# BetterBelle/eco-dqn

Measured on NVIDIA B200. Metric: env-steps/sec incl. MPNN Q-eval, higher is better.
Workload: dtype bf16x2-split/f32

## Files before the change

### eco-dqn_b200/csrc/env_step_device.cuh

```cuda
#pragma once
#include <limits.h>

#include "eco_common.cuh"

namespace eco {

union V8s { uint2 v; int8_t b[8]; };
union V8h { uint4 v; int16_t h[8]; };
union V8u { uint4 v; uint16_t h[8]; };
union V4s { uint32_t v; int8_t b[4]; };
union V4h { uint2 v; int16_t h[4]; };
union V4u { uint2 v; uint16_t h[4]; };

__device__ __forceinline__ float feat_gain(int gain, double mlr) {
    return (float)__ddiv_rn((double)gain, mlr);
}

struct SmallDiv {
    float m, y;
    bool ok;
};
__device__ __forceinline__ SmallDiv small_div_setup(double mlr, bool integer_couplings) {
    SmallDiv d;
    d.m = (float)mlr;
    d.ok = integer_couplings && mlr != 0.0 && fabs(mlr) <= 2048.0;
    d.y = __frcp_rn(d.ok ? d.m : 1.f);
    return d;
}
__device__ __forceinline__ float small_div(float a, const SmallDiv& d) {
    const float q0 = __fmul_rn(a, d.y);
    const float r = __fmaf_rn(-q0, d.m, a);
    return __fmaf_rn(r, d.y, q0);
}
__device__ __forceinline__ uint32_t prmt(uint32_t a, uint32_t b, uint32_t sel) {
    uint32_t r;
    asm("prmt.b32 %0, %1, %2, %3;" : "=r"(r) : "r"(a), "r"(b), "r"(sel));
    return r;
}
__device__ __forceinline__ int sx8(uint32_t w, int k) { return (int)prmt(w, 0, k | ((8 | k) << 4) | ((8 | k) << 8) | ((8 | k) << 12)); }
__device__ __forceinline__ int sx16(uint32_t w, int hh) {
    return (int)prmt(w, 0, (2 * hh) | ((2 * hh + 1) << 4) | ((8 | (2 * hh + 1)) << 8) | ((8 | (2 * hh + 1)) << 12));
}
__device__ __forceinline__ int zx16(uint32_t w, int hh) { return (int)prmt(w, 0, (2 * hh) | ((2 * hh + 1) << 4) | 0x4400); }

struct StepScalars {
    double score, nscore, best_score, best_nscore, rew;
    int n_visited;
    bool new_best;
};
__device__ __forceinline__ StepScalars bls_step_scalars(const eco_env_t& env, const double (&sc)[4], double delta,
                                                        double delta_n, int nimp, int n_visited, uint64_t* tab, uint32_t slot,
                                                        ulonglong2 tv, uint64_t k0, uint64_t k1) {
    StepScalars r;
    r.score = __dadd_rn(sc[0], delta);
    r.nscore = __dadd_rn(sc[1], delta_n);
    r.rew = 0.0;
    if (r.score > sc[2]) r.rew = __dsub_rn(r.nscore, sc[3]);
    if (env.use_basin) {
        const uint64_t w0 = k0 ^ VISITED_SALT0, w1 = k1 ^ VISITED_SALT1;
        bool is_new = false;
        for (int probe = 0; probe < env.HCAP; ++probe) {
            if (tv.x == 0 && tv.y == 0) {
                *reinterpret_cast<ulonglong2*>(tab + 2 * slot) = make_ulonglong2(w0, w1);
                is_new = true; ++n_visited;
                break;
            }
            if (tv.x == w0 && tv.y == w1) break;
            slot = (slot + 1) & (env.HCAP - 1);
            tv = *reinterpret_cast<const ulonglong2*>(tab + 2 * slot);
        }
        if (nimp == 0 && is_new) r.rew = __dadd_rn(r.rew, env.basin_reward);
    }
    r.n_visited = n_visited;
    r.new_best = r.score > sc[2];
    r.best_score = r.new_best ? r.score : sc[2];
    r.best_nscore = r.new_best ? r.nscore : sc[3];
    return r;
}

template <int TPE, bool WIDE = true>
__device__ __forceinline__ void env_step_group(const eco_graphs_t& g, const eco_env_t& env, long long b, const int lane,
                                               const bool in_range, const int policy, const int action,
                                               double* __restrict__ reward_out, uint8_t* __restrict__ done_out,
                                               int32_t* __restrict__ hist_a, double* __restrict__ hist_r,
                                               double* __restrict__ hist_s) {
    const int N = env.N, NP = env.NP, NCH = NP >> 3;
    const bool has = lane < NCH;

    eco_episode_t* ep = env.ep + b;
    const int4 e0 = *reinterpret_cast<const int4*>(ep);
    const int4 e1 = *(reinterpret_cast<const int4*>(ep) + 1);
    const int gi = env.graph_idx[b];
    int a = policy == ECO_POLICY_GREEDY ? 0 : action;
    int8_t* spins = env.spins + (size_t)b * NP;
    int16_t* hf = env.hfield + (size_t)b * NP;
    uint16_t* lf = env.last_flip + (size_t)b * NP;
    V8s s; V8h h; V8u l;
    s.v = make_uint2(0, 0); h.v = make_uint4(0, 0, 0, 0); l.v = make_uint4(0, 0, 0, 0);
    if (has) {
        s.v = *reinterpret_cast<const uint2*>(spins + lane * 8);
        h.v = *reinterpret_cast<const uint4*>(hf + lane * 8);
        l.v = *reinterpret_cast<const uint4*>(lf + lane * 8);
    }
    double sc[4] = {0, 0, 0, 0};
    ulonglong2 key = make_ulonglong2(0, 0);
    double total_reward = 0.0;
    if (lane == 0) {
        const double2 d0 = *reinterpret_cast<const double2*>(&ep->score);
        const double2 d1 = *reinterpret_cast<const double2*>(&ep->best_score);
        sc[0] = d0.x; sc[1] = d0.y; sc[2] = d1.x; sc[3] = d1.y;
        key = *reinterpret_cast<const ulonglong2*>(&ep->key[0]);
        total_reward = ep->total_reward;
    }
    const int flags = e1.y;
    const int step_new = e0.x + 1;
    bool active = in_range && !(flags & (FLAG_DONE | FLAG_STOPPED)) && step_new <= env.T;

    if (policy == ECO_POLICY_GREEDY) {
        int best = INT_MIN;
#pragma unroll
        for (int k = 0; k < 8; ++k) {
            const int i = lane * 8 + k;
            if (has && i < N)
                best = max(best, (int)((((uint32_t)(s.b[k] * h.h[k] + 32768) << 16) | (uint32_t)(0xFFFF - i)) ^ 0x80000000u));
        }
        best = group_max<TPE>(best);
        const uint32_t ukey = (uint32_t)best ^ 0x80000000u;
        a = 0xFFFF - (int)(ukey & 0xFFFFu);
        if (active && ((int)(ukey >> 16) - 32768) < 0) {
            active = false;
            if (lane == 0) ep->flags = flags | FLAG_STOPPED;
        }
    }
    if (a < 0 || a >= N) { a = 0; active = false; }

    V8s j;
    j.v = make_uint2(0, 0);
    if (has && active) j.v = *reinterpret_cast<const uint2*>(g.J + ((size_t)gi * NP + a) * NP + lane * 8);
    const double mlr = g.gscal[(size_t)gi * 4 + 0];
    const bool use_tab = (g.reserved & ECO_GRAPHS_PM1) != 0;
    const float* gtab = g.gain_tab + (size_t)gi * tab_stride(NP) + NP;
    double qn = 1.0;
    ulonglong2 zob = make_ulonglong2(0, 0);
    uint32_t old_word = 0;
    if (lane == 0) {
        if (!use_tab) qn = g.gscal[(size_t)gi * 4 + 1];
        zob = *reinterpret_cast<const ulonglong2*>(env.zobrist + 2 * a);
        old_word = env.diff_bits[(size_t)b * env.NW + (a >> 5)];
    }
    const int ka = a & 7;
    const uint32_t sw = ka < 4 ? s.v.x : s.v.y;
    const int my_s = (int)(int8_t)(sw >> (8 * (ka & 3)));
    const uint32_t hw = ka < 2 ? h.v.x : (ka < 4 ? h.v.y : (ka < 6 ? h.v.z : h.v.w));
    const int my_h = (int)(int16_t)(hw >> (16 * (ka & 1)));
    const int s_a_old = __shfl_sync(0xffffffffu, my_s, a >> 3, TPE);
    const int h_a_old = __shfl_sync(0xffffffffu, my_h, a >> 3, TPE);
    const int s_a_new = -s_a_old;

    const uint64_t k0 = key.x ^ zob.x, k1 = key.y ^ zob.y;
    uint64_t* tab = env.visited + (size_t)b * env.HCAP * 2;
    uint32_t slot = (uint32_t)(k0 ^ (k0 >> 29)) & (env.HCAP - 1);
    ulonglong2 tv = make_ulonglong2(0, 0);
    const int delta = s_a_old * h_a_old;
    double delta_n = 0.0;
    if (lane == 0 && active) {
        if (env.use_basin) tv = *reinterpret_cast<const ulonglong2*>(tab + 2 * slot);
        if (use_tab) delta_n = __ldg(g.dn_tab + (size_t)gi * tab_stride(NP) + NP + delta);
    }

    int nimp = 0;
    if (has && active) {
        float* x0 = env.xn + (size_t)b * 3 * NP + lane * 8;
        auto vertex = [&](int k, float& o0, float& o1, float& o2) {
            const int i = lane * 8 + k;
            int si = s.b[k];
            if (i == a) { si = s_a_new; s.b[k] = (int8_t)si; l.h[k] = (uint16_t)step_new; }
            const int hi = h.h[k] + 2 * j.b[k] * s_a_new;
            h.h[k] = (int16_t)hi;
            const int gain = si * hi;
            nimp += gain > 0;
            o0 = (float)si;
            o1 = use_tab ? __ldg(gtab + gain) : feat_gain(gain, mlr);
            o2 = __ldg(env.tsf_tab + (step_new - l.h[k]));
        };
        if (WIDE) {
            float f0[8], f1[8], f2[8];
#pragma unroll
            for (int k = 0; k < 8; ++k) vertex(k, f0[k], f1[k], f2[k]);
            st_f32x8(x0, f0);
            st_f32x8(x0 + NP, f1);
            st_f32x8(x0 + 2 * NP, f2);
        } else {
#pragma unroll
            for (int half = 0; half < 2; ++half) {
                float f0[4], f1[4], f2[4];
#pragma unroll
                for (int kk = 0; kk < 4; ++kk) vertex(half * 4 + kk, f0[kk], f1[kk], f2[kk]);
                *reinterpret_cast<float4*>(x0 + 4 * half) = make_float4(f0[0], f0[1], f0[2], f0[3]);
                *reinterpret_cast<float4*>(x0 + NP + 4 * half) = make_float4(f1[0], f1[1], f1[2], f1[3]);
// ... 53 lines not shown
```

### eco-dqn_b200/csrc/mpnn_tc.cu

```cuda
#include <cuda_bf16.h>
#include <stdlib.h>

#include "eco_common.cuh"
#include "tc_prims.cuh"
#include "mpnn_pack.cuh"
#include "env_step_device.cuh"

namespace eco {
namespace {

using namespace tc;

constexpr int NPMAX = 208;
constexpr int PACK_NPMAX = 192;
constexpr int CHUNK = 64;
constexpr int SUBS = 2;
constexpr int THREADS = 256 * SUBS;
constexpr int GROUP_THREADS = 128 * SUBS;
constexpr int NWARPS = THREADS / 32;
constexpr int ISSUERS = 4;
constexpr int LAUNCH_THREADS = THREADS + 32 * ISSUERS;

constexpr uint32_t T_ACC0 = 0;
constexpr uint32_t T_ACC1 = 208;
// ... 116 lines not shown
}

__device__ __forceinline__ void store_block(const Ctx& c, unsigned char* buf, int node0, const float (&v)[8]) {
    const int rowoff = 16 * (c.lane >> 2) + 4 * (c.lane & 3);
#pragma unroll
    for (int half = 0; half < 2; ++half) {
        const int cb = (node0 >> 3) + half;
#pragma unroll
        for (int fr = 0; fr < 2; ++fr) {
            uint32_t hi, lo;
            split2(v[4 * half + 2 * fr], v[4 * half + 2 * fr + 1], hi, lo);
            unsigned char* p = buf + ((cb * 16 + 4 * c.q + fr) * 128) + rowoff;
            *reinterpret_cast<uint32_t*>(p) = hi;
            *reinterpret_cast<uint32_t*>(p + 2 * 128) = lo;
        }
    }
}

__device__ __forceinline__ void issue_part(const Ctx& c, uint32_t acc_col, uint32_t tw, const unsigned char* x, int cb0,
                                           int width , bool accumulate) {
    const uint32_t idesc = instr_desc_bf16(128, width, false, true);
    const uint32_t idesc_lo = instr_desc_bf16(64, width, false, true);
    const uint64_t d = smem_desc(smem_u32(x) + cb0 * 2048,  128,  2048);
#pragma unroll
    for (int i = 0; i < 8; ++i)
        mma_ts(c.tmem + acc_col, c.tmem + tw + 8 * (i >> 1), d + (uint64_t)(16 * i), (i & 1) ? idesc_lo : idesc, accumulate || i > 0);
}

struct FusedEnv {
    eco_env_t env;
    int32_t* hist_a;
    double* hist_r;
    double* hist_s;
    int n_steps;
};

template <bool PACKED, bool TLINE, bool FUSED = false>
__global__ void __launch_bounds__(LAUNCH_THREADS, 1)
mpnn_tc_kernel(const eco_graphs_t g, const eco_mpnn_t w, const int B, const int32_t* __restrict__ graph_idx,
               const float* __restrict__ xn, const float* __restrict__ xg, const float norm_max,
               float* __restrict__ q_out, int32_t* __restrict__ act_out, unsigned long long* __restrict__ dbg,
               const int packK, const FusedEnv fe) {
    extern __shared__ __align__(128) unsigned char smem[];
    int dbg_n = 0;
#define TL(id)                                                                                           \
    do {                                                                                                 \
        if (TLINE && dbg != nullptr && blockIdx.x == 0 && (threadIdx.x & 31) == 0 && dbg_n < 1024)       \
            dbg[(threadIdx.x >> 5) * 1024 + dbg_n++] = ((unsigned long long)(id) << 48) | (clock64() & 0xFFFFFFFFFFFFull); \
    } while (0)
    __shared__ uint64_t bars[9];
    __shared__ uint64_t sig[2];
    __shared__ uint64_t sdbar[4];
    __shared__ uint64_t tail_sig, tail_done;
    __shared__ uint64_t gsig[2][2];
    __shared__ uint64_t bar_ops[2];
    __shared__ uint32_t tmem_base_s;
    Ctx c;
    c.smem = smem; c.phase_all = 0; c.phase_grp = 0; c.phase_g2 = 0; c.phase_g3 = 0;
    c.tid = threadIdx.x; c.lane = c.tid & 31;
    c.warp = __shfl_sync(0xffffffffu, c.tid >> 5, 0);
    c.q = c.warp & 3; c.sub = (c.warp >> 2) % SUBS;
    c.grp = c.warp < NWARPS ? c.warp / (4 * SUBS) : (c.warp == NWARPS + 2 ? 1 : 0);
    const bool linear_issuer = c.warp == NWARPS + 1 || c.warp == NWARPS + 2;
    c.bar_all = &bars[0]; c.bar_grp = &bars[1 + c.grp]; c.bar_g2 = &bars[5 + c.grp]; c.bar_g3 = &bars[7 + c.grp];
    const int K = PACKED ? packK : 1;
    const int NPs = g.NP, Ns = g.N;
    c.NP = K * NPs; c.NB = c.NP >> 3; c.N = PACKED ? c.NP : g.N;
    const int N = c.N, NP = c.NP, NB = c.NB;
    const int N8 = PACKED ? NP : ((N + 7) & ~7);
    const int npacks = (B + K - 1) / K;
    const int n_e = (int)blockIdx.x < npacks ? (npacks - (int)blockIdx.x + (int)gridDim.x - 1) / (int)gridDim.x : 0;
    const int n_items = n_e * (FUSED ? fe.n_steps : 1);
    auto item_ep = [&](int it) { return (int)blockIdx.x + (FUSED ? it % n_e : it) * (int)gridDim.x; };
    auto vertex_ok = [&](int n) { return PACKED ? (n % NPs) < Ns : n < N; };
    float* rdmaxv = reinterpret_cast<float*>(smem + SM_A + PACK_NPMAX * PACK_NPMAX * 2);
    float* pp_blk = rdmaxv + PACK_NPMAX;
    float* pooled_e = pp_blk + (PACK_NPMAX / 16) * 64;
    float* tef = pooled_e + (PACK_NPMAX / 16) * 64;

    float* xf = reinterpret_cast<float*>(smem + SM_XF);
    float* rdeg = reinterpret_cast<float*>(smem + SM_DEG);
    float* qpart = reinterpret_cast<float*>(smem + SM_QP);
    float* ppart = reinterpret_cast<float*>(smem + SM_PP);
    float* pooled = ppart;
    float* s_c0 = reinterpret_cast<float*>(smem + SM_MISC);
    float* red_val = s_c0 + 16;
    int* red_idx = reinterpret_cast<int*>(s_c0 + 32);
    unsigned char* sA = smem + SM_A;
    unsigned char* sAbs = smem + SM_ABS;
    unsigned char* sH = smem + SM_H;
    unsigned char* sE = smem + SM_E;
    unsigned char* sT = smem + SM_T + c.grp * (128 * CHUNK * 2);
    const uint32_t acc1 = T_ACC1 + 64 * c.grp;
    const uint32_t* pk = reinterpret_cast<const uint32_t*>(w.packed);

    if (c.warp == 0) tmem_alloc(&tmem_base_s, 512);
    if (c.tid == 0) {
        for (int i = 0; i < 9; ++i) mbar_init(&bars[i], 1);
        mbar_init(&bar_ops[0], 1); mbar_init(&bar_ops[1], 1);
        mbar_init(&sig[0], 1); mbar_init(&sig[1], 1);
        for (int i = 0; i < 4; ++i) mbar_init(&gsig[i >> 1][i & 1], 4 * SUBS);
        for (int i = 0; i < 4; ++i) mbar_init(&sdbar[i], NWARPS);
        mbar_init(&tail_sig, 1); mbar_init(&tail_done, 1);
        fence_mbar_init();
    }
    tc_fence_before();
    __syncthreads();
    tc_fence_after();
    c.tmem = tmem_base_s;
    if (c.warp < 4 && N8 < NP) {
        const uint32_t z[8] = {0, 0, 0, 0, 0, 0, 0, 0};
        tmem_st_32x32b_x8(tmem_addr(c.tmem, 32 * c.q, T_ACC0 + N8), z);
        tmem_st_wait();
        tc_fence_before();
    }
    const float dmax_set = norm_max > 0.f ? norm_max : *g.dmax;
    const int nsteps_A = NP >> 4;
    const int nblocks = NP >> 4;
    const int nb0 = group0_blocks(nblocks), nb1 = nblocks - nb0;
    const int nch0 = nb0 >= 2 ? 2 : nb0, nch1 = nb1 >= 2 ? 2 : nb1;
    const int nchunks = nch0 + nch1;
    const int chunk_split = nch0;
    const int cs = c.grp == 0 ? 0 : nch0;
    const int ncols0 = 16 * nb0;
    uint32_t phase_half = 0, phase_other = 0, phase_tail = 0;
    const int nmine = (c.warp < NWARPS || linear_issuer) ? (c.grp == 0 ? nch0 : nch1) : 0;
    const int nbm = c.grp == 0 ? nb0 : nb1;
    const int cA0 = c.grp == 0 ? 0 : ncols0, cAw = nmine > 1 ? 16 * ((nbm + 1) / 2) : 16 * nbm;
    const int cB0 = cA0 + cAw, cBw = 16 * nbm - cAw;
    const int cAm = min(cAw, N8 - cA0), cBm = min(cBw, N8 - cB0);
    auto signal_issuer = [&](int k) {
        fence_proxy_async();
        tc_fence_before();
        __syncwarp();
        if (c.lane == 0) mbar_arrive(&gsig[c.grp][k & 1]);
    };

// ... 88 lines not shown
            for (int j = 0; j < 16; ++j) {
                const float pv = pooled[k0 + 2 * j + kpar];
                acc.x = fmaf(a[j].x, pv, acc.x); acc.y = fmaf(a[j].y, pv, acc.y);
                acc.z = fmaf(a[j].z, pv, acc.z); acc.w = fmaf(a[j].w, pv, acc.w);
            }
        }
        acc.x += __shfl_xor_sync(0xffffffffu, acc.x, 16); acc.y += __shfl_xor_sync(0xffffffffu, acc.y, 16);
        acc.z += __shfl_xor_sync(0xffffffffu, acc.z, 16); acc.w += __shfl_xor_sync(0xffffffffu, acc.w, 16);
        const float4 wr = __ldg(reinterpret_cast<const float4*>(w.w_read + f4));
        float t = kpar == 0 ? fmaf(wr.x, fmaxf(acc.x, 0.f), fmaf(wr.y, fmaxf(acc.y, 0.f),
                              fmaf(wr.z, fmaxf(acc.z, 0.f), wr.w * fmaxf(acc.w, 0.f)))) : 0.f;
#pragma unroll
        for (int o = 16; o > 0; o >>= 1) t += __shfl_xor_sync(0xffffffffu, t, o);
        TL(62);
        return bread + t;
    };
    auto readout_warp_b = [&](const int be, const float c0v) {
        TL(63);
        float bv = -INFINITY;
        int bi = 0x7fffffff;
        for (int i = c.lane; i < N; i += 32) {
            const float qv = c0v + ((qpart[i] + qpart[NPMAX + i]) + (qpart[2 * NPMAX + i] + qpart[3 * NPMAX + i]));
            if (q_out) q_out[(size_t)be * NP + i] = qv;
            if (qv > bv) { bv = qv; bi = i; }
        }
#pragma unroll
        for (int o = 16; o > 0; o >>= 1) {
            const float ov = __shfl_xor_sync(0xffffffffu, bv, o);
            const int oi = __shfl_xor_sync(0xffffffffu, bi, o);
            if (ov > bv || (ov == bv && oi < bi)) { bv = ov; bi = oi; }
        }
        if (c.lane == 0 && act_out) act_out[be] = bi;
        if (FUSED)
            env_step_group<32, false>(g, fe.env, be, c.lane, true, ECO_POLICY_ACTIONS, bi, nullptr, nullptr, fe.hist_a, fe.hist_r, fe.hist_s);
        TL(64);
    };
    constexpr int XF_DEG = 4, XF_GL = 5, XF_GMAX = 6;
    float* wsm_e = xf + 7 * NPMAX;
    float* wsm_i = wsm_e + 63 * 8;
    auto stage_inputs = [&](int e) {
        const int i = c.tid - GROUP_THREADS, per_row = NP >> 2;
        const int ge = graph_idx[e];
        if (i < 4 * per_row) {
            const int row = i / per_row, col = 4 * (i % per_row);
            const float* src = row < 3 ? xn + ((size_t)e * 3 + row) * NP + col : g.deg + (size_t)ge * NP + col;
            float* dst = xf + (row < 3 ? row : XF_DEG) * NPMAX + col;
            asm volatile("cp.async.cg.shared.global [%0], [%1], 16;" ::"r"(smem_u32(dst)), "l"(src) : "memory");
        } else if (i == 4 * per_row) {
            asm volatile("cp.async.cg.shared.global [%0], [%1], 16;" ::"r"(smem_u32(xf + XF_GL * NPMAX)), "l"(xg + (size_t)e * 4) : "memory");
        } else if (i == 4 * per_row + 1) {
            asm volatile("cp.async.ca.shared.global [%0], [%1], 4;" ::"r"(smem_u32(xf + XF_GMAX * NPMAX)), "l"(g.gstat + (size_t)ge * 4) : "memory");
        }
        if (i < (63 * 8) / 4)
            asm volatile("cp.async.ca.shared.global [%0], [%1], 16;" ::"r"(smem_u32(wsm_e + 4 * i)), "l"(w.w_edge + 4 * i) : "memory");
        if (i < (64 * 7) / 4)
            asm volatile("cp.async.ca.shared.global [%0], [%1], 16;" ::"r"(smem_u32(wsm_i + 4 * i)), "l"(w.w_init + 4 * i) : "memory");
        asm volatile("cp.async.commit_group;" ::: "memory");
    };
    auto readout_packed_warp = [&](const int be) {
        TL(60);
        const int bpe = NPs >> 4;
        for (int idx = c.lane; idx < K * 64; idx += 32) {
            const int e = idx >> 6, f = idx & 63;
            float t = 0.f;
            for (int j = 0; j < bpe; ++j) t += pp_blk[(e * bpe + j) * 64 + f];
            pooled_e[idx] = t / (float)Ns;
        }
        __syncwarp();
        TL(61);
        constexpr int KMAX = PACK_NPMAX / 16;
        float p0[KMAX], p1[KMAX];
#pragma unroll
        for (int e = 0; e < KMAX; ++e) { p0[e] = 0.f; p1[e] = 0.f; }
        const float* wt = reinterpret_cast<const float*>(pk + PK_WPT) + c.lane;
#pragma unroll 1
        for (int k0 = 0; k0 < 64; k0 += 16) {
            float wa[16], wb[16];
#pragma unroll
            for (int j = 0; j < 16; ++j) { wa[j] = __ldg(wt + (k0 + j) * 64); wb[j] = __ldg(wt + (k0 + j) * 64 + 32); }
#pragma unroll
            for (int j = 0; j < 16; ++j) {
#pragma unroll
                for (int e = 0; e < KMAX; ++e) {
                    if (e < K) {
                        const float pv = pooled_e[e * 64 + k0 + j];
                        p0[e] = fmaf(wa[j], pv, p0[e]);
                        p1[e] = fmaf(wb[j], pv, p1[e]);
                    }
                }
            }
        }
// ... 19 lines not shown
            const int ep = be * K + e;
            const float c0v = pooled_e[e];
            for (int v = c.lane; v < NPs; v += 32) {
                const int i = i0 + v;
                const float qv = c0v + ((qpart[i] + qpart[NPMAX + i]) + (qpart[2 * NPMAX + i] + qpart[3 * NPMAX + i]));
                const bool ok = v < Ns && ep < B;
                if (ok && q_out) q_out[(size_t)ep * NPs + v] = qv;
                qpart[i] = ok ? qv : -INFINITY;
            }
        }
        __syncwarp();
        TL(65);
        for (int e = 0; e < K; ++e) {
            const int ep = be * K + e;
            float bv = -INFINITY;
            int bi = 0x7fffffff;
            for (int v = c.lane; v < Ns; v += 32) {
                const float qv = qpart[e * NPs + v];
                if (qv > bv) { bv = qv; bi = v; }
            }
#pragma unroll
            for (int o = 16; o > 0; o >>= 1) {
                const float ov = __shfl_xor_sync(0xffffffffu, bv, o);
                const int oi = __shfl_xor_sync(0xffffffffu, bi, o);
                if (ov > bv || (ov == bv && oi < bi)) { bv = ov; bi = oi; }
            }
            if (c.lane == 0 && ep < B && act_out) act_out[ep] = bi;
        }
        TL(64);
    };
    if (c.warp == NWARPS) {

        uint32_t sp0 = 0, sp1 = 0, sp2 = 0, op = 0;
        for (int it = 0; it < n_items; ++it) {
            mbar_wait(&bar_ops[0], op);
            mbar_wait(&bar_ops[1], op); op ^= 1u;
            TL(51);
            for (int r = 0; 4 * r < nsteps_A; ++r) {
                mbar_wait(&sdbar[r], sp0);
                tc_fence_after();
                if (r == 0) TL(50);
                if (elect_one()) {
                    const uint32_t idesc = instr_desc_bf16(128, N8, false, false);
                    const uint64_t bd_abs = smem_desc(smem_u32(sAbs), NB * 128, 128);
                    const uint64_t bd_a = smem_desc(smem_u32(sA), NB * 128, 128);
                    const uint64_t kstep = (uint64_t)((2 * NB * 128) >> 4);
                    for (int ks = 4 * r; ks < min(4 * r + 4, nsteps_A); ++ks) {
                        mma_ts(c.tmem + T_ACC0, c.tmem + T_S + 8 * ks, bd_abs + ks * kstep, idesc, ks > 0);
                        mma_ts(c.tmem + T_ACC0, c.tmem + T_D + 8 * ks, bd_a + ks * kstep, idesc, true);
                    }
                    if (4 * r + 4 >= nsteps_A) mma_commit(c.bar_all);
                }
                __syncwarp();
            }
            sp0 ^= 1u;
            TL(52);
            for (int l = 0; l < 3; ++l) {
                mbar_wait(&sig[1], sp1); sp1 ^= 1u;
                tc_fence_after();
                TL(53);
                if (elect_one()) {
                    const uint64_t ad = smem_desc(smem_u32(sH), 2048, 128);
                    const uint64_t bstep = (uint64_t)((2 * NB * 128) >> 4);
                    for (int half = 0; half < 2; ++half) {
                        const int n0 = half ? ncols0 : 0, ncols = half ? N8 - ncols0 : min(ncols0, N8);
                        if (ncols == 0) break;
                        const uint32_t idesc = instr_desc_bf16(128, ncols, false, false);
                        const uint64_t bd = smem_desc(smem_u32(sA) + (n0 >> 3) * 128, NB * 128, 128);
                        for (int ks = 0; ks < nsteps_A; ++ks)
                            mma_ss(c.tmem + T_ACC0 + n0, ad + (uint64_t)ks * (4096 >> 4), bd + ks * bstep, idesc, ks > 0);
                        mma_commit(&bars[3 + half]);
                    }
                }
                __syncwarp();
                TL(54);
            }
            if (PACKED && it + 1 < n_items) {
                mbar_wait(&bars[N8 > ncols0 ? 4 : 3], (uint32_t)((3 * it + 2) & 1));
                fetch_ops_warp(0, item_ep(it + 1));
                mbar_wait(&sig[0], sp2); sp2 ^= 1u;
                fetch_ops_warp(1, item_ep(it + 1));
            }
        }
    }
    if (c.warp == NWARPS + 3) {
        uint32_t ph = 0;
        for (int it = 0; it < n_items - (PACKED ? 1 : 0); ++it) {
            mbar_wait(&tail_sig, ph);
            ph ^= 1u;
            if (PACKED) readout_packed_warp(item_ep(it));
            else readout_warp_b(item_ep(it), readout_warp_a());
            if (FUSED) __threadfence();
            __syncwarp();
            if (c.lane == 0) mbar_arrive(&tail_done);
        }
    }
    if (linear_issuer && nmine > 0) {
        uint32_t ph[2] = {0, 0};
        auto wait_sig = [&](int k) {
            mbar_wait(&gsig[c.grp][k & 1], ph[k & 1]);
            ph[k & 1] ^= 1u;
            tc_fence_after();
        };
        for (int it = 0; it < n_items; ++it) {
            wait_sig(0);
            if (elect_one()) { issue_part(c, T_ACC0 + cA0, T_WEF, sE, cA0 >> 3, cAm, false); mma_commit(c.bar_grp); }
            __syncwarp();
            if (nmine > 1) {
                wait_sig(1);
                if (elect_one()) { issue_part(c, acc1, T_WEF, sE, cB0 >> 3, cBm, false); mma_commit(c.bar_g2); }
                __syncwarp();
            }
            for (int l = 0; l < 3; ++l) {
                wait_sig(0);
                if (elect_one()) issue_part(c, acc1, T_WM + 32, sE, cA0 >> 3, cAm, false);
                __syncwarp();
                wait_sig(1);
                if (elect_one()) {
                    issue_part(c, acc1, T_WM, sT, 0, cAm, true);
                    mma_commit(c.bar_grp);
                    issue_part(c, T_ACC0 + cA0, T_WU, sH, cA0 >> 3, cAm, false);
                    mma_commit(c.bar_g2);
                }
                __syncwarp();
                if (nmine > 1) {
                    wait_sig(0);
                    if (elect_one()) {
                        issue_part(c, T_ACC0 + cB0, T_WU, sH, cB0 >> 3, cBm, false);
                        mma_commit(c.bar_g3);
                    }
                    __syncwarp();
                }
                wait_sig(1);
                if (elect_one()) {
                    issue_part(c, T_ACC0 + cA0, T_WU + 32, sH, cA0 >> 3, cAm, true);
                    mma_commit(c.bar_grp);
                    if (nmine > 1) {
// ... 45 lines not shown
            workers_sync();
            if (c.tid < NP) {
                const int i = c.tid, e = i / NPs, v = i % NPs, ep = be * K + e;
                float c0v = bread;
                for (int f = 0; f < 64; ++f) c0v += tef[e * 64 + f];
                const float qv = c0v + ((qpart[i] + qpart[NPMAX + i]) + (qpart[2 * NPMAX + i] + qpart[3 * NPMAX + i]));
                const bool ok = v < Ns && ep < B;
                if (ok && q_out) q_out[(size_t)ep * NPs + v] = qv;
                qpart[i] = ok ? qv : -INFINITY;
            }
            workers_sync();
            for (int e = c.warp; e < K; e += NWARPS) {
                const int ep = be * K + e;
                float bv = -INFINITY;
                int bi = 0x7fffffff;
                for (int v = c.lane; v < Ns; v += 32) {
                    const float qv = qpart[e * NPs + v];
                    if (qv > bv) { bv = qv; bi = v; }
                }
#pragma unroll
                for (int o = 16; o > 0; o >>= 1) {
                    const float ov = __shfl_xor_sync(0xffffffffu, bv, o);
                    const int oi = __shfl_xor_sync(0xffffffffu, bi, o);
                    if (ov > bv || (ov == bv && oi < bi)) { bv = ov; bi = oi; }
                }
                if (c.lane == 0 && ep < B && act_out) act_out[ep] = bi;
            }
            workers_sync();
            return;
        }
    };
    int last_b = -1;

    for (int it = 0; it < n_items && c.warp < NWARPS; ++it) {
        const int b = item_ep(it);
        const bool has_next = it + 1 < n_items;
        const int b_next = has_next ? item_ep(it + 1) : 0;
        TL(1);
        if (!PACKED) {
            asm volatile("cp.async.wait_group 0;" ::: "memory");
            TL(70);
            workers_sync();
            TL(71);
            gl = *reinterpret_cast<const float4*>(xf + XF_GL * NPMAX);
            gmaxdeg = *reinterpret_cast<const int*>(xf + XF_GMAX * NPMAX);
            if (has_v) rdeg[c.tid] = __fdividef(1.f, xf[XF_DEG * NPMAX + c.tid]);
        }
        const float rdmax = __fdividef(1.f, norm_max < 0.f ? (float)max(gmaxdeg, 1) : dmax_set);

        const int fa = 16 * c.q + (c.lane >> 2), fb = fa + 8;
        float wxa[8], wxb[8], wia[7], wib[7];
        {
            const float* we = PACKED ? w.w_edge : wsm_e;
            const float* wi = PACKED ? w.w_init : wsm_i;
#pragma unroll
            for (int k = 0; k < 8; ++k) {
                wxa[k] = we[fa * 8 + k];
                wxb[k] = fb < 63 ? we[fb * 8 + k] : 0.f;
            }
#pragma unroll
            for (int k = 0; k < 7; ++k) { wia[k] = wi[fa * 7 + k]; wib[k] = wi[fb * 7 + k]; }
        }
        if (PACKED && has_v) {
            const int i = c.tid;
            const bool ok = vertex_ok(i);
            xf[0 * NPMAX + i] = ok ? xin0 : 0.f;
            xf[1 * NPMAX + i] = ok ? xin1 : 0.f;
            xf[2 * NPMAX + i] = ok ? xin2 : 0.f;
            rdeg[i] = __fdividef(1.f, degv);
            {
                xf[3 * NPMAX + i] = ok ? gl.x : 0.f;
                xf[4 * NPMAX + i] = ok ? gl.y : 0.f;
                xf[5 * NPMAX + i] = ok ? gl.z : 0.f;
                xf[6 * NPMAX + i] = ok ? gl.w : 0.f;
                rdmaxv[i] = 1.f / (norm_max < 0.f ? (float)max(gmaxdeg, 1) : dmax_set);
            }
// ... 116 lines not shown
                store_block(c, sE, c0 + bc, v);
            });
        };
        if (nmine > 0) {
            TL(15);
            wait_grp(c);
            TL(12);
            epi_e(T_ACC0, cA0, cA0, cAw);
            TL(13);
        }

        auto epi_agg = [&](int c0, int width, bool wait_b1) {
            bool waited = !wait_b1;
            epilogue(c, T_ACC0, c0, width, [&](int bc, float (&v)[8]) {
                const int n0 = c0 + bc + 2 * (c.lane & 3);
                const float2 r0 = *reinterpret_cast<const float2*>(rdeg + n0), r1 = *reinterpret_cast<const float2*>(rdeg + n0 + 8);
                const float rd[4] = {r0.x, r0.y, r1.x, r1.y};
#pragma unroll
                for (int i = 0; i < 8; i += 2) mul2(v[i], v[i + 1], v[i], v[i + 1], rd[2 * (i >> 2)], rd[2 * (i >> 2) + 1]);
                if (!waited) { wait_grp(c); waited = true; }
                store_block(c, sT, bc, v);
            });
            if (!waited) wait_grp(c);
        };
        auto epi_m = [&](int c0, int width) {
            epilogue(c, acc1, 0, width, [&](int bc, float (&v)[8]) {
#pragma unroll
                for (int i = 0; i < 8; ++i) v[i] = fmaxf(v[i], 0.f);
                store_block(c, sH, c0 + bc, v);
            });
        };
        for (int l = 0; l < 3; ++l) {
            TL(20);
            cta_stage_sync();
            TL(21);
            if (c.tid == 0) mbar_arrive(&sig[1]);
            if (l > 0) {
                uint4 wm[64 / (8 * SUBS)], wu[64 / (8 * SUBS)];
                ldg_weights<64>(c, pk + PK_WM + l * 128 * 64, wm);
                ldg_weights<64>(c, pk + PK_WU + l * 128 * 64, wu);
                sttm_weights<64>(c, wm, T_WM);
                sttm_weights<64>(c, wu, T_WU);
                tmem_st_wait();
                tc_fence_before();
                workers_sync();
            }
            if (l == 0 && nmine > 1) {
                wait_g2(c);
                epi_e(acc1, 0, cB0, cBw);
                TL(13);
            }
            if (nmine > 0) signal_issuer(0);
            TL(22);
            float wa = 0.f, wb = 0.f;
            if (l == 2) { wa = __ldg(w.w_read + 64 + fa); wb = __ldg(w.w_read + 64 + fa + 8); }
            if (l == 2 && last_b >= 0) {
                mbar_wait(&tail_done, phase_tail);
                phase_tail ^= 1u;
            }
            if (nmine > 0) {
                mbar_wait(&bars[3 + c.grp], phase_half);
                phase_half ^= 1u;
                tc_fence_after();
            }
            TL(23);
            if (!PACKED && l == 2 && c.tid == (chunk_split < nchunks ? THREADS / 2 : 0) && has_next) fetch_ops(0, b_next);
            auto epi_h = [&](int ci, int c0, int width) {
                if (l < 2) {
// ... 40 lines not shown
                pool_b += __shfl_xor_sync(0xffffffffu, pool_b, 1); pool_b += __shfl_xor_sync(0xffffffffu, pool_b, 2);
                if (!PACKED && (c.lane & 3) == 0) {
                    ppart[(ci * SUBS + c.sub) * 64 + fa] = pool_a;
                    ppart[(ci * SUBS + c.sub) * 64 + fa + 8] = pool_b;
                }
            };
            if (nmine > 0) {
                epi_agg(cA0, cAw, false);
                signal_issuer(1);
                TL(30);
                if (nmine > 1) {
                    epi_agg(cB0, cBw, true);
                    signal_issuer(0);
                    TL(31);
                } else {
                    wait_grp(c);
                }
                wait_g2(c);
                if (c.grp == 0 && chunk_split < nchunks) {
                    mbar_wait(&bars[4], phase_other);
                    phase_other ^= 1u;
                }
                TL(33);
                epi_m(cA0, cAw);
                signal_issuer(1);
                TL(34);
                wait_grp(c);
                TL(37);
                epi_h(cs, cA0, cAw);
                TL(38);
                if (nmine > 1) {
                    wait_g2(c);
                    wait_g3(c);
                    if (!PACKED && l == 2 && c.grp == 1 && has_next) stage_inputs(b_next);
                    TL(33);
                    epi_m(cB0, cBw);
                    signal_issuer(0);
                    TL(35);
                    wait_grp(c);
                    TL(37);
                    epi_h(cs + 1, cB0, cBw);
                    TL(38);
                }
            }
        }
        TL(40);

        if (has_next) {
            if (PACKED) load_inputs(b_next);
            else if (c.grp == 1 && nmine < 2) stage_inputs(b_next);
        }
        workers_sync();
        if (PACKED && has_next) {
            TL(42);
            zero_image(smem + SM_ABS);
            workers_sync();
            TL(43);
        }
        if (c.tid == 0 && has_next) {
            if (PACKED) mbar_arrive(&sig[0]);
            else fetch_ops(1, b_next);
        }
        if (c.tid == 0 && (!PACKED || has_next)) mbar_arrive(&tail_sig);
        last_b = b;
        TL(41);
    }
    if (PACKED && c.warp < NWARPS && last_b >= 0) readout_packed_all(last_b);
#undef TL

    tc_fence_before();
    __syncthreads();
    if (c.warp == 0) tmem_dealloc(c.tmem, 512);
}

}

bool mpnn_tc_supported(const eco_graphs_t* g) { return g->N <= NPMAX && (g->reserved & ECO_GRAPHS_PM1) && g->tc_ops != nullptr; }
size_t mpnn_tc_scratch_bytes(int, int) { return (NWARPS + ISSUERS) * 1024 * 8 + 256; }
size_t mpnn_tc_packed_bytes() { return (size_t)PK_WORDS * 4; }

int launch_mpnn_pack(const eco_mpnn_t* w, void* packed, cudaStream_t st) {
    mpnn_pack_kernel<<<(PK_WORDS + 255) / 256, 256, 0, st>>>(*w, (uint32_t*)packed);
    ECO_LAUNCH_CHECK();
    return ECO_OK;
}

bool mpnn_tc_can_fuse(const eco_graphs_t* g, const eco_env_t* env) {
    const bool packed = PACK_NPMAX / g->NP >= 2 && env->B >= 2;
    return mpnn_tc_supported(g) && !packed && env->reserved == 0 && !(g->reserved & ECO_GRAPHS_MIN_CUT) && env->N == g->N &&
           env->B >= 2 * device_sm_count();
}

int launch_mpnn_tc(const eco_graphs_t* g, const eco_mpnn_t* w, int B, const int32_t* gidx, const float* xn,
                   const float* xg, float norm_max, float* q, int32_t* actions, void* scratch, cudaStream_t st) {
    return launch_mpnn_tc_fused(g, w, B, gidx, xn, xg, norm_max, q, actions, scratch, nullptr, 1, nullptr, nullptr, nullptr, st);
}

int launch_mpnn_tc_fused(const eco_graphs_t* g, const eco_mpnn_t* w, int B, const int32_t* gidx, const float* xn,
                         const float* xg, float norm_max, float* q, int32_t* actions, void* scratch, const eco_env_t* fused,
                         int n_steps, int32_t* ha, double* hr, double* hs, cudaStream_t st) {
    static unsigned long long attr_set = 0;
    const int n_sm = device_sm_count();
    if (first_use_on_device(&attr_set)) {
        ECO_CUDA((cudaFuncSetAttribute(mpnn_tc_kernel<false, false>, cudaFuncAttributeMaxDynamicSharedMemorySize, SM_TOTAL)));
        ECO_CUDA((cudaFuncSetAttribute(mpnn_tc_kernel<true, false>, cudaFuncAttributeMaxDynamicSharedMemorySize, SM_TOTAL)));
        ECO_CUDA((cudaFuncSetAttribute(mpnn_tc_kernel<false, true>, cudaFuncAttributeMaxDynamicSharedMemorySize, SM_TOTAL)));
        ECO_CUDA((cudaFuncSetAttribute(mpnn_tc_kernel<true, true>, cudaFuncAttributeMaxDynamicSharedMemorySize, SM_TOTAL)));
        ECO_CUDA((cudaFuncSetAttribute(mpnn_tc_kernel<false, false, true>, cudaFuncAttributeMaxDynamicSharedMemorySize, SM_TOTAL)));
    }
    const int packK = PACK_NPMAX / g->NP;
    const bool packed = packK >= 2 && B >= 2;
    if (fused && packed) { set_error("launch_mpnn_tc_fused: packed batches cannot be fused"); return ECO_ERR_INVALID; }
    const int units = packed ? (B + packK - 1) / packK : B;
    const int grid = units < n_sm ? units : n_sm;
    const int prof_kind = fused ? ECO_PROF_ROLLOUT : ECO_PROF_MPNN;
    prof_begin(prof_kind, st, fused ? n_steps : 1);
    static const bool timeline = getenv("ECO_TC_TIMELINE") != nullptr;
    if (timeline) ECO_CUDA(cudaMemsetAsync(scratch, 0, (NWARPS + ISSUERS) * 1024 * 8, st));
    unsigned long long* dbg = timeline ? (unsigned long long*)scratch : nullptr;
    FusedEnv fe{};
    fe.n_steps = 1;
    if (fused) {
        if (n_steps < 1 || B < 2 * grid) { set_error("launch_mpnn_tc_fused: needs n_steps >= 1 and two episodes per CTA"); return ECO_ERR_INVALID; }
        fe.env = *fused; fe.hist_a = ha; fe.hist_r = hr; fe.hist_s = hs; fe.n_steps = n_steps;
    }
    if (packed && dbg) mpnn_tc_kernel<true, true><<<grid, LAUNCH_THREADS, SM_TOTAL, st>>>(*g, *w, B, gidx, xn, xg, norm_max, q, actions, dbg, packK, fe);
    else if (packed) mpnn_tc_kernel<true, false><<<grid, LAUNCH_THREADS, SM_TOTAL, st>>>(*g, *w, B, gidx, xn, xg, norm_max, q, actions, nullptr, packK, fe);
    else if (dbg) mpnn_tc_kernel<false, true><<<grid, LAUNCH_THREADS, SM_TOTAL, st>>>(*g, *w, B, gidx, xn, xg, norm_max, q, actions, dbg, 1, fe);
    else if (fused) mpnn_tc_kernel<false, false, true><<<grid, LAUNCH_THREADS, SM_TOTAL, st>>>(*g, *w, B, gidx, xn, xg, norm_max, q, actions, nullptr, 1, fe);
    else mpnn_tc_kernel<false, false><<<grid, LAUNCH_THREADS, SM_TOTAL, st>>>(*g, *w, B, gidx, xn, xg, norm_max, q, actions, nullptr, 1, fe);
    prof_end(prof_kind, st);
    ECO_LAUNCH_CHECK();
    return ECO_OK;
}

}
```

Measured before the change: 7.679 million.

## Dynamically schedule fused rollout work items across CTAs via global claim counter

Replaces the static round-robin episode×step assignment in the fused MPNN+env-step kernel with a global atomic work counter, a small per-CTA ring of claimed items, and per-episode publication flags using acquire/release. A CTA can therefore pick up any episode whose previous step has been published, instead of waiting on its fixed episodes. Env state loads switch to L2-cached (__ldcg) reads because other SMs now write that state. The cost is atomics, spin-waiting with nanosleep on cross-CTA dependencies, an extra memset per launch, and splitting very long rollouts into several launches.

```diff
diff --git a/eco-dqn_b200/csrc/env_step_device.cuh b/eco-dqn_b200/csrc/env_step_device.cuh
--- a/eco-dqn_b200/csrc/env_step_device.cuh
+++ b/eco-dqn_b200/csrc/env_step_device.cuh
@@ -42,6 +42,12 @@
     return (int)prmt(w, 0, (2 * hh) | ((2 * hh + 1) << 4) | ((8 | (2 * hh + 1)) << 8) | ((8 | (2 * hh + 1)) << 12));
 }
 __device__ __forceinline__ int zx16(uint32_t w, int hh) { return (int)prmt(w, 0, (2 * hh) | ((2 * hh + 1) << 4) | 0x4400); }
+
+template <bool CG, class T>
+__device__ __forceinline__ T ld_state(const T* p) {
+    if constexpr (CG) return __ldcg(p);
+    else return *p;
+}
 
 struct StepScalars {
     double score, nscore, best_score, best_nscore, rew;
@@ -78,7 +84,7 @@
     return r;
 }
 
-template <int TPE, bool WIDE = true>
+template <int TPE, bool WIDE = true, bool CG = false>
 __device__ __forceinline__ void env_step_group(const eco_graphs_t& g, const eco_env_t& env, long long b, const int lane,
                                                const bool in_range, const int policy, const int action,
                                                double* __restrict__ reward_out, uint8_t* __restrict__ done_out,
@@ -88,8 +94,8 @@
     const bool has = lane < NCH;
 
     eco_episode_t* ep = env.ep + b;
-    const int4 e0 = *reinterpret_cast<const int4*>(ep);
-    const int4 e1 = *(reinterpret_cast<const int4*>(ep) + 1);
+    const int4 e0 = ld_state<CG>(reinterpret_cast<const int4*>(ep));
+    const int4 e1 = ld_state<CG>(reinterpret_cast<const int4*>(ep) + 1);
     const int gi = env.graph_idx[b];
     int a = policy == ECO_POLICY_GREEDY ? 0 : action;
     int8_t* spins = env.spins + (size_t)b * NP;
@@ -98,19 +104,19 @@
     V8s s; V8h h; V8u l;
     s.v = make_uint2(0, 0); h.v = make_uint4(0, 0, 0, 0); l.v = make_uint4(0, 0, 0, 0);
     if (has) {
-        s.v = *reinterpret_cast<const uint2*>(spins + lane * 8);
-        h.v = *reinterpret_cast<const uint4*>(hf + lane * 8);
-        l.v = *reinterpret_cast<const uint4*>(lf + lane * 8);
+        s.v = ld_state<CG>(reinterpret_cast<const uint2*>(spins + lane * 8));
+        h.v = ld_state<CG>(reinterpret_cast<const uint4*>(hf + lane * 8));
+        l.v = ld_state<CG>(reinterpret_cast<const uint4*>(lf + lane * 8));
     }
     double sc[4] = {0, 0, 0, 0};
     ulonglong2 key = make_ulonglong2(0, 0);
     double total_reward = 0.0;
     if (lane == 0) {
-        const double2 d0 = *reinterpret_cast<const double2*>(&ep->score);
-        const double2 d1 = *reinterpret_cast<const double2*>(&ep->best_score);
+        const double2 d0 = ld_state<CG>(reinterpret_cast<const double2*>(&ep->score));
+        const double2 d1 = ld_state<CG>(reinterpret_cast<const double2*>(&ep->best_score));
         sc[0] = d0.x; sc[1] = d0.y; sc[2] = d1.x; sc[3] = d1.y;
-        key = *reinterpret_cast<const ulonglong2*>(&ep->key[0]);
-        total_reward = ep->total_reward;
+        key = ld_state<CG>(reinterpret_cast<const ulonglong2*>(&ep->key[0]));
+        total_reward = ld_state<CG>(&ep->total_reward);
     }
     const int flags = e1.y;
     const int step_new = e0.x + 1;
@@ -146,7 +152,7 @@
     if (lane == 0) {
         if (!use_tab) qn = g.gscal[(size_t)gi * 4 + 1];
         zob = *reinterpret_cast<const ulonglong2*>(env.zobrist + 2 * a);
-        old_word = env.diff_bits[(size_t)b * env.NW + (a >> 5)];
+        old_word = ld_state<CG>(env.diff_bits + (size_t)b * env.NW + (a >> 5));
     }
     const int ka = a & 7;
     const uint32_t sw = ka < 4 ? s.v.x : s.v.y;
@@ -164,7 +170,7 @@
     const int delta = s_a_old * h_a_old;
     double delta_n = 0.0;
     if (lane == 0 && active) {
-        if (env.use_basin) tv = *reinterpret_cast<const ulonglong2*>(tab + 2 * slot);
+        if (env.use_basin) tv = ld_state<CG>(reinterpret_cast<const ulonglong2*>(tab + 2 * slot));
         if (use_tab) delta_n = __ldg(g.dn_tab + (size_t)gi * tab_stride(NP) + NP + delta);
     }
 
diff --git a/eco-dqn_b200/csrc/mpnn_tc.cu b/eco-dqn_b200/csrc/mpnn_tc.cu
--- a/eco-dqn_b200/csrc/mpnn_tc.cu
+++ b/eco-dqn_b200/csrc/mpnn_tc.cu
@@ -172,6 +172,7 @@
     int32_t* hist_a;
     double* hist_r;
     double* hist_s;
+    uint32_t* claim;
     int n_steps;
 };
 
@@ -210,8 +211,12 @@
     const int N8 = PACKED ? NP : ((N + 7) & ~7);
     const int npacks = (B + K - 1) / K;
     const int n_e = (int)blockIdx.x < npacks ? (npacks - (int)blockIdx.x + (int)gridDim.x - 1) / (int)gridDim.x : 0;
-    const int n_items = n_e * (FUSED ? fe.n_steps : 1);
-    auto item_ep = [&](int it) { return (int)blockIdx.x + (FUSED ? it % n_e : it) * (int)gridDim.x; };
+    const int n_items = n_e;
+    auto item_ep = [&](int it) { return (int)blockIdx.x + it * (int)gridDim.x; };
+    const int n_total = FUSED ? B * fe.n_steps : 0;
+    int* ring = reinterpret_cast<int*>(smem + SM_MISC);
+    uint64_t* pub_bar = reinterpret_cast<uint64_t*>(smem + SM_MISC + 16);
+    auto has_item = [&](int it) { return __all_sync(0xffffffffu, ring[it & 3] < n_total); };
     auto vertex_ok = [&](int n) { return PACKED ? (n % NPs) < Ns : n < N; };
     float* rdmaxv = reinterpret_cast<float*>(smem + SM_A + PACK_NPMAX * PACK_NPMAX * 2);
     float* pp_blk = rdmaxv + PACK_NPMAX;
@@ -223,9 +228,6 @@
     float* qpart = reinterpret_cast<float*>(smem + SM_QP);
     float* ppart = reinterpret_cast<float*>(smem + SM_PP);
     float* pooled = ppart;
-    float* s_c0 = reinterpret_cast<float*>(smem + SM_MISC);
-    float* red_val = s_c0 + 16;
-    int* red_idx = reinterpret_cast<int*>(s_c0 + 32);
     unsigned char* sA = smem + SM_A;
     unsigned char* sAbs = smem + SM_ABS;
     unsigned char* sH = smem + SM_H;
@@ -242,7 +244,9 @@
         for (int i = 0; i < 4; ++i) mbar_init(&gsig[i >> 1][i & 1], 4 * SUBS);
         for (int i = 0; i < 4; ++i) mbar_init(&sdbar[i], NWARPS);
         mbar_init(&tail_sig, 1); mbar_init(&tail_done, 1);
+        if (FUSED) mbar_init(pub_bar, 1);
         fence_mbar_init();
+        if (FUSED) ring[0] = blockIdx.x;
     }
     tc_fence_before();
     __syncthreads();
@@ -397,7 +401,8 @@
         }
         if (c.lane == 0 && act_out) act_out[be] = bi;
         if (FUSED)
-            env_step_group<32, false>(g, fe.env, be, c.lane, true, ECO_POLICY_ACTIONS, bi, nullptr, nullptr, fe.hist_a, fe.hist_r, fe.hist_s);
+            env_step_group<32, false, true>(g, fe.env, be, c.lane, true, ECO_POLICY_ACTIONS, bi, nullptr, nullptr, fe.hist_a, fe.hist_r,
+                                            fe.hist_s);
         TL(64);
     };
     constexpr int XF_DEG = 4, XF_GL = 5, XF_GMAX = 6;
@@ -422,6 +427,18 @@
             asm volatile("cp.async.ca.shared.global [%0], [%1], 16;" ::"r"(smem_u32(wsm_i + 4 * i)), "l"(w.w_init + 4 * i) : "memory");
         asm volatile("cp.async.commit_group;" ::: "memory");
     };
+    auto published = [&](int k) {
+        const int s = k / B;
+        uint32_t v = 0;
+        if (s > 0) asm volatile("ld.acquire.gpu.global.u32 %0, [%1];" : "=r"(v) : "l"(fe.claim + 1 + (k - s * B)) : "memory");
+        return __all_sync(0xffffffffu, (int)v >= s);
+    };
+    bool stage_late = false;
+    uint32_t pub_ph = 0;
+    auto stage_next = [&](int e) {
+        if (mbar_test(pub_bar, pub_ph)) { pub_ph ^= 1u; stage_inputs(e); }
+        else stage_late = true;
+    };
     auto readout_packed_warp = [&](const int be) {
         TL(60);
         const int bpe = NPs >> 4;
@@ -507,7 +524,7 @@
     if (c.warp == NWARPS) {
 
         uint32_t sp0 = 0, sp1 = 0, sp2 = 0, op = 0;
-        for (int it = 0; it < n_items; ++it) {
+        for (int it = 0; FUSED ? has_item(it) : it < n_items; ++it) {
             mbar_wait(&bar_ops[0], op);
             mbar_wait(&bar_ops[1], op); op ^= 1u;
             TL(51);
@@ -550,6 +567,14 @@
                 __syncwarp();
                 TL(54);
             }
+            if (FUSED && has_item(it + 1)) {
+                for (uint32_t n = 0; !published(ring[(it + 1) & 3]); ++n) {
+                    if (n > (1u << 24)) __trap();
+                    __nanosleep(256);
+                }
+                if (c.lane == 0) mbar_arrive(pub_bar);
+                __syncwarp();
+            }
             if (PACKED && it + 1 < n_items) {
                 mbar_wait(&bars[N8 > ncols0 ? 4 : 3], (uint32_t)((3 * it + 2) & 1));
                 fetch_ops_warp(0, item_ep(it + 1));
@@ -560,13 +585,16 @@
     }
     if (c.warp == NWARPS + 3) {
         uint32_t ph = 0;
-        for (int it = 0; it < n_items - (PACKED ? 1 : 0); ++it) {
+        for (int it = 0; FUSED ? has_item(it) : it < n_items - (PACKED ? 1 : 0); ++it) {
             mbar_wait(&tail_sig, ph);
             ph ^= 1u;
+            const int k = FUSED ? ring[it & 3] : 0, s = k / B;
             if (PACKED) readout_packed_warp(item_ep(it));
-            else readout_warp_b(item_ep(it), readout_warp_a());
+            else readout_warp_b(FUSED ? k - s * B : item_ep(it), readout_warp_a());
             if (FUSED) __threadfence();
             __syncwarp();
+            if (FUSED && c.lane == 0)
+                asm volatile("st.relaxed.gpu.global.u32 [%0], %1;" ::"l"(fe.claim + 1 + (k - s * B)), "r"(s + 1) : "memory");
             if (c.lane == 0) mbar_arrive(&tail_done);
         }
     }
@@ -577,7 +605,7 @@
             ph[k & 1] ^= 1u;
             tc_fence_after();
         };
-        for (int it = 0; it < n_items; ++it) {
+        for (int it = 0; FUSED ? has_item(it) : it < n_items; ++it) {
             wait_sig(0);
             if (elect_one()) { issue_part(c, T_ACC0 + cA0, T_WEF, sE, cA0 >> 3, cAm, false); mma_commit(c.bar_grp); }
             __syncwarp();
@@ -689,16 +717,24 @@
     };
     int last_b = -1;
 
-    for (int it = 0; it < n_items && c.warp < NWARPS; ++it) {
-        const int b = item_ep(it);
-        const bool has_next = it + 1 < n_items;
-        const int b_next = has_next ? item_ep(it + 1) : 0;
+    for (int it = 0; (FUSED ? has_item(it) : it < n_items) && c.warp < NWARPS; ++it) {
+        const int k = FUSED ? ring[it & 3] : 0;
+        const int b = FUSED ? k % B : item_ep(it);
+        bool has_next = !FUSED && it + 1 < n_items;
+        int b_next = has_next ? item_ep(it + 1) : 0, claim = 0;
         TL(1);
+        if (FUSED && stage_late) {
+            mbar_wait(pub_bar, pub_ph);
+            pub_ph ^= 1u;
+            stage_inputs(b);
+            stage_late = false;
+        }
         if (!PACKED) {
             asm volatile("cp.async.wait_group 0;" ::: "memory");
             TL(70);
             workers_sync();
             TL(71);
+            if (FUSED && c.tid == 0) claim = (int)gridDim.x + (int)atomicAdd(fe.claim, 1u);
             gl = *reinterpret_cast<const float4*>(xf + XF_GL * NPMAX);
             gmaxdeg = *reinterpret_cast<const int*>(xf + XF_GMAX * NPMAX);
             if (has_v) rdeg[c.tid] = __fdividef(1.f, xf[XF_DEG * NPMAX + c.tid]);
@@ -881,8 +917,14 @@
         };
         for (int l = 0; l < 3; ++l) {
             TL(20);
+            if (FUSED && l == 0 && c.tid == 0) ring[(it + 1) & 3] = claim;
             cta_stage_sync();
             TL(21);
+            if (FUSED && l == 2) {
+                const int k_next = ring[(it + 1) & 3];
+                has_next = k_next < n_total;
+                b_next = k_next % B;
+            }
             if (c.tid == 0) mbar_arrive(&sig[1]);
             if (l > 0) {
                 uint4 wm[64 / (8 * SUBS)], wu[64 / (8 * SUBS)];
@@ -989,7 +1031,10 @@
                 if (nmine > 1) {
                     wait_g2(c);
                     wait_g3(c);
-                    if (!PACKED && l == 2 && c.grp == 1 && has_next) stage_inputs(b_next);
+                    if (!PACKED && l == 2 && c.grp == 1 && has_next) {
+                        if (FUSED) stage_next(b_next);
+                        else stage_inputs(b_next);
+                    }
                     TL(33);
                     epi_m(cB0, cBw);
                     signal_issuer(0);
@@ -1005,7 +1050,10 @@
 
         if (has_next) {
             if (PACKED) load_inputs(b_next);
-            else if (c.grp == 1 && nmine < 2) stage_inputs(b_next);
+            else if (c.grp == 1 && nmine < 2) {
+                if (FUSED) stage_next(b_next);
+                else stage_inputs(b_next);
+            }
         }
         workers_sync();
         if (PACKED && has_next) {
@@ -1033,7 +1081,8 @@
 }
 
 bool mpnn_tc_supported(const eco_graphs_t* g) { return g->N <= NPMAX && (g->reserved & ECO_GRAPHS_PM1) && g->tc_ops != nullptr; }
-size_t mpnn_tc_scratch_bytes(int, int) { return (NWARPS + ISSUERS) * 1024 * 8 + 256; }
+constexpr size_t TIMELINE_BYTES = (NWARPS + ISSUERS) * 1024 * 8;
+size_t mpnn_tc_scratch_bytes(int B, int) { return TIMELINE_BYTES + 256 + (size_t)4 * (B + 1); }
 size_t mpnn_tc_packed_bytes() { return (size_t)PK_WORDS * 4; }
 
 int launch_mpnn_pack(const eco_mpnn_t* w, void* packed, cudaStream_t st) {
@@ -1073,18 +1122,27 @@
     const int prof_kind = fused ? ECO_PROF_ROLLOUT : ECO_PROF_MPNN;
     prof_begin(prof_kind, st, fused ? n_steps : 1);
     static const bool timeline = getenv("ECO_TC_TIMELINE") != nullptr;
-    if (timeline) ECO_CUDA(cudaMemsetAsync(scratch, 0, (NWARPS + ISSUERS) * 1024 * 8, st));
+    if (timeline) ECO_CUDA(cudaMemsetAsync(scratch, 0, TIMELINE_BYTES, st));
     unsigned long long* dbg = timeline ? (unsigned long long*)scratch : nullptr;
     FusedEnv fe{};
     fe.n_steps = 1;
     if (fused) {
         if (n_steps < 1 || B < 2 * grid) { set_error("launch_mpnn_tc_fused: needs n_steps >= 1 and two episodes per CTA"); return ECO_ERR_INVALID; }
         fe.env = *fused; fe.hist_a = ha; fe.hist_r = hr; fe.hist_s = hs; fe.n_steps = n_steps;
-    }
+        fe.claim = reinterpret_cast<uint32_t*>(static_cast<char*>(scratch) + TIMELINE_BYTES + 256);
+    }
+    const int max_steps = fused ? (int)((0x7fffffffll - grid) / B) : 1;
     if (packed && dbg) mpnn_tc_kernel<true, true><<<grid, LAUNCH_THREADS, SM_TOTAL, st>>>(*g, *w, B, gidx, xn, xg, norm_max, q, actions, dbg, packK, fe);
     else if (packed) mpnn_tc_kernel<true, false><<<grid, LAUNCH_THREADS, SM_TOTAL, st>>>(*g, *w, B, gidx, xn, xg, norm_max, q, actions, nullptr, packK, fe);
     else if (dbg) mpnn_tc_kernel<false, true><<<grid, LAUNCH_THREADS, SM_TOTAL, st>>>(*g, *w, B, gidx, xn, xg, norm_max, q, actions, dbg, 1, fe);
-    else if (fused) mpnn_tc_kernel<false, false, true><<<grid, LAUNCH_THREADS, SM_TOTAL, st>>>(*g, *w, B, gidx, xn, xg, norm_max, q, actions, nullptr, 1, fe);
+    else if (fused) {
+        for (int s0 = 0; s0 < n_steps; s0 += max_steps) {
+            fe.n_steps = n_steps - s0 < max_steps ? n_steps - s0 : max_steps;
+            ECO_CUDA(cudaMemsetAsync(fe.claim, 0, (size_t)4 * (B + 1), st));
+            mpnn_tc_kernel<false, false, true><<<grid, LAUNCH_THREADS, SM_TOTAL, st>>>(*g, *w, B, gidx, xn, xg, norm_max, q, actions,
+                                                                                       nullptr, 1, fe);
+        }
+    }
     else mpnn_tc_kernel<false, false><<<grid, LAUNCH_THREADS, SM_TOTAL, st>>>(*g, *w, B, gidx, xn, xg, norm_max, q, actions, nullptr, 1, fe);
     prof_end(prof_kind, st);
     ECO_LAUNCH_CHECK();
```

Measured after the change: 7.636 million (median of 6 runs). Within noise of the previous version (-0.6%).
